# ariasanovsky/azdopt

Measured on AMD Instinct MI355X. Metric: node_expansions_per_s, higher is better.
Workload: dtype f32

## Files before the change

### azdopt_amd/_lib.py

```python
import ctypes as C
import os
import subprocess

_HERE = os.path.dirname(os.path.abspath(__file__))
LIB_PATH = os.environ.get("AZD_LIB", os.path.join(_HERE, "libazdopt_amd.so"))
_LIB = None

CTR = dict(EXPANSIONS=0, TERMINALS=1, TRANSPOSITIONS=2, VISITED_STEPS=3, SELECT_CALLS=4, SUM_DEG=5,
           SUM_ACTIONS=6, CASCADE_NODES=7, NEW_PREDS=8, ROOT_EXHAUSTED=9, MAX_FRONTIER=10, MAX_DEPTH=11,
           CURIOSITY_PAIRS=12, EVAL_LAYER_CLOCKS=13, TICKS_ADD_ACTIONS=14, FAILED=15, TICKS_TOTAL=16, TICKS_SELECT=17, TICKS_LOOKUP=18, TICKS_NEWNODE=19,
           TICKS_CASCADE=20, TICKS_MAX_CALL=21, TICKS_LAMBDA=22, TICKS_MATCHING=23, TICKS_WAIT=24, EVAL_BATCHES=25, EVAL_ROWS=26, EVAL_TILES=27, TICKS_TILES=28, TICKS_BATCH=29, TICKS_TILE_SETUP=30, TICKS_TILE_KLOOP=31)
CTR_COUNT = 32

ACT_NONE, ACT_RELU, ACT_SIGMOID = 0, 1, 2
ENGINE_NO_PERSISTENT_STEP = 1
ENGINE_ASYNC_STEP = 2
ENGINE_BARRIER_STEP = 4
ENGINE_POOL_STEP = 8
ENGINE_DENSE_AH = 32
ENGINE_RAMSEY_U64 = 16
ENGINE_EXT_POOL_STEP = 64
ENGINE_EXT_POOL_F32 = 128
SPACE_C21 = 1
SPACE_RAMSEY = 2
# ... 98 lines not shown
    sig("azd_version", C.c_int)
    sig("azd_device_count", C.c_int)
    sig("azd_c21_state_dim", C.c_int, C.c_int)
    sig("azd_c21_action_dim", C.c_int, C.c_int)
    sig("azd_c21_key_words", C.c_int, C.c_int)
    sig("azd_c21_generate_roots", C.c_int, C.c_uint64, C.c_uint64, C.c_uint64, C.c_int, C.c_int, C.c_int, C.c_int, vp, vp)
    sig("azd_evaluator_create_mlp", C.c_int, C.POINTER(vp), C.c_int, C.c_int, C.c_int, C.c_int, vp, C.c_int, C.c_int,
        C.POINTER(AdamConfig), C.c_uint64)
    sig("azd_evaluator_create_trivial", C.c_int, C.POINTER(vp), C.c_int, C.c_int, C.c_int)
    sig("azd_evaluator_create_hash_stream", C.c_int, C.POINTER(vp), C.c_int, C.c_int, C.c_int, C.c_uint64, C.c_uint64)
    sig("azd_evaluator_destroy", C.c_int, vp)
    sig("azd_evaluator_write_predictions", C.c_int, vp, C.c_int, vp, vp)
    sig("azd_evaluator_update_model", C.c_int, vp, C.c_int, vp, vp, vp, f32p)
    sig("azd_evaluator_write_predictions_dev", C.c_int, vp, C.c_int, vp, vp, vp)
    sig("azd_evaluator_update_model_dev", C.c_int, vp, C.c_int, vp, vp, vp, f32p, vp)
    sig("azd_evaluator_set_weight_storage", C.c_int, vp, C.c_int)
    sig("azd_evaluator_num_params", C.c_int64, vp)
    sig("azd_evaluator_get_params", C.c_int, vp, vp)
    sig("azd_evaluator_set_params", C.c_int, vp, vp)
    sig("azd_evaluator_calls", C.c_uint64, vp)
    sig("azd_engine_create", C.c_int, C.POINTER(vp), C.POINTER(EngineConfig), vp)
    sig("azd_engine_destroy", C.c_int, vp)
    sig("azd_engine_par_new", C.c_int, vp, vp, vp)
    sig("azd_engine_par_roll_out_episodes", C.c_int, vp, vp, C.c_int, C.c_uint32, C.c_int, i32p)
    sig("azd_engine_run_ahead", C.c_int, vp, vp, C.c_int, C.c_uint32, C.c_int, i32p)
    sig("azd_engine_par_update_model", C.c_int, vp, C.c_uint32, f32p)
    sig("azd_engine_par_update_model_sharded", C.c_int, vp, C.c_uint32, vp, f32p)
    sig("azd_engine_par_reset_trees", C.c_int, vp, vp, vp)
    sig("azd_engine_argmin_data", C.c_int, vp, C.POINTER(Argmin))
    sig("azd_engine_agent_counters", C.c_int, vp, vp)
    sig("azd_engine_agent_counters_per_agent", C.c_int, vp)
    sig("azd_engine_pool_agent_finish", C.c_int, vp, vp)
    sig("azd_engine_pool_groups", C.c_int, vp, vp, vp, vp)
    sig("azd_engine_ramsey_argmin_data", C.c_int, vp, C.POINTER(RamseyArgmin))
    sig("azd_engine_ramsey_wide_argmin_data", C.c_int, vp, C.POINTER(RamseyWideArgmin))
    sig("azd_engine_ramsey_argmin_any", C.c_int, vp, vp, C.c_int, vp, C.c_int, vp, f32p, i32p, C.POINTER(C.c_uint32))
    sig("azd_engine_ramsey_agent_counts", C.c_int, vp, C.c_int, vp, vp)
    sig("azd_ramsey_state_dim", C.c_int, C.c_int, C.c_int)
    sig("azd_ramsey_action_dim", C.c_int, C.c_int, C.c_int)
    sig("azd_ramsey_key_words", C.c_int, C.c_int, C.c_int)
    sig("azd_ramsey_generate_roots", C.c_int, C.c_uint64, C.c_uint64, C.c_uint64, C.c_int, C.c_int, C.c_int, C.c_int,
        C.c_int, vp, vp)
    sig("azd_ramsey_generate_roots_weighted", C.c_int, C.c_uint64, C.c_uint64, C.c_uint64, C.c_int, C.c_int, C.c_int, C.c_int,
        C.c_int, vp, vp, vp)
    sig("azd_engine_set_root_policy", C.c_int, vp, C.POINTER(RootPolicy))
    sig("azd_engine_get_root_policy", C.c_int, vp, C.POINTER(RootPolicy))
    sig("azd_root_policy_check", C.c_int, C.c_int, C.c_int, C.POINTER(RootPolicy))
    sig("azd_engine_root_policy_report", C.c_int, vp, vp, vp, vp)
    sig("azd_dense_state_dim", C.c_int, C.c_int)
    sig("azd_dense_action_dim", C.c_int, C.c_int)
    sig("azd_dense_key_words", C.c_int, C.c_int)
    sig("azd_dense_generate_roots", C.c_int, C.c_uint64, C.c_uint64, C.c_uint64, C.c_int, C.c_int, C.c_int, C.c_int, C.c_double, vp, vp)
    sig("azd_engine_dense_argmin_data", C.c_int, vp, C.POINTER(DenseArgmin))
    sig("azd_c21_modify_roots", C.c_int, vp, C.c_uint64, C.c_uint64, C.c_int, C.c_int, vp, vp)
    sig("azd_c21_modify_roots_dev", C.c_int, vp, C.c_uint64, C.c_uint64, C.c_int, C.c_int, vp, vp)
    sig("azd_engine_par_reset_trees_c21", C.c_int, vp, C.c_uint64, C.c_uint64, C.c_int, C.c_int)
    sig("azd_engine_modify_roots_dev", C.c_int, vp, C.c_uint64, C.c_uint64, C.c_int, C.c_int, vp, vp)
    sig("azd_engine_par_reset_trees_policy", C.c_int, vp, C.c_uint64, C.c_uint64, C.c_int, C.c_int)
    sig("azd_engine_par_new_begin", C.c_int, vp, vp, vp)
    sig("azd_engine_par_new_end", C.c_int, vp, vp)
    sig("azd_engine_roll_out_begin", C.c_int, vp, vp, C.c_int, C.c_uint32)
    sig("azd_engine_roll_out_end", C.c_int, vp, vp, i32p)
    sig("azd_engine_reset_begin", C.c_int, vp, vp, vp)
    sig("azd_engine_reset_end", C.c_int, vp, vp)
    sig("azd_engine_observe", C.c_int, vp, C.c_uint32, vp, vp, vp)
    sig("azd_engine_observe_dev", C.c_int, vp, C.c_uint32, C.POINTER(vp), C.POINTER(vp), C.POINTER(vp))
# ... 38 lines not shown
```

### azdopt_amd/csrc/engine.hip

```cpp
#include <hip/hip_runtime.h>

#include <dlfcn.h>

#include <algorithm>
#include <climits>
#include <cstdio>
#include <cstring>
#include <functional>
#include <new>
#include <string>
#include <vector>

#include "../../include/azdopt_amd.h"
#include "c21_host.h"
#include "engine_types.h"
#include "evaluator.h"
#include "space_ops.h"

namespace azd {

thread_local std::string g_last_error;

int hip_fail(hipError_t e, const char *what) {
    g_last_error = std::string(what) + ": " + hipGetErrorString(e);
// ... 200 lines not shown
    static constexpr int EXT_STREAMS = 2;
    static constexpr int EXT_IN_FLIGHT = 4;
    hipStream_t ext_stream[EXT_STREAMS] = {};
    hipGraphExec_t ext_graph[EXT_STREAMS] = {};
    uint64_t ext_graph_layout = 0;
    int ext_graph_n = 0;
    bool ext_unsupported = false;
    bool ext_f32 = false;
    uint64_t ext_unsupported_layout = 0;
    uint32_t *d_ext_rows = nullptr, *d_ext_home = nullptr, *d_ext_n = nullptr;
    unsigned long long *d_ext_t0 = nullptr;
    int ext_depth = 2;
    hipEvent_t ext_done = nullptr, ext_fork = nullptr, ext_ring[EXT_STREAMS][EXT_IN_FLIGHT] = {};
    unsigned long long ext_iterations = 0;
    const struct ExtPoolForm *ext = nullptr;
    uint16_t *ext_s16 = nullptr;
    int ext_s16_pitch = 0;
    int kw_host = 0;
    int ramsey_slots = 0;
    int dense_slots = 0;
    uint64_t *d_stage_slots = nullptr;
    azd_root_policy root_policy{AZD_ROOT_RULE_THRESHOLD, 0, {0.0, 0.0, 0.0, 0.0}};
    azd::RootPolicyArgs root_args{};
    uint32_t *d_root_report = nullptr;
    uint32_t *root_report = nullptr;
    bool root_report_valid = false;
    std::vector<uint64_t> dense_packed;
    std::vector<uint64_t> ramsey_perm_pad;
    bool pool_step = false;
    azd::PoolArgs pool{};
    size_t pool_slot_words = 0;
    int n_cus = 0;
    int pool_eval_wgs = 0, pool_search_wgs = 0;
    int pool_grp_g = 0, pool_grp_groups = 0, pool_grp_w = 0;
    int pool_search_waves = 0;
    double pool_util_eval = 0, pool_util_search = 0;
    struct {
        int n_eval = 0;
        int updates = 0;
    } pool_fb;
    struct Window {
        bool open = false;
        bool drained = false;
        bool lumped = false;
        int n = 0, consumed = 0;
        azd::TolTable tol{};
        uint32_t best_ord = 0;
        unsigned long long best_key = ~0ull;
        unsigned long long side_key = ~0ull;
        unsigned long long base_improved = 0;
        unsigned long long reported = 0;
        azd::FusedEval fe{};
        azd::PoolArgs pool{};
    } win;
    unsigned long long *h_win_log = nullptr;
    uint32_t *h_win_flag = nullptr;
    azd::ArgminRec *d_argmin_side = nullptr;
    azd::RamseyArgminRec *d_argmin_r_side = nullptr;
    bool ramsey_wide() const { return a.space == azd::SPACE_RAMSEY && a.KW > azd::MAX_KW; }
    bool dense_ah() const { return a.space == azd::SPACE_DENSE && a.lam_lo != 0.0; }
    bool ramsey_u64() const { return a.space == azd::SPACE_RAMSEY && a.KW == azd::RAMSEY_U64_KW; }
    size_t ramsey_nbr_words() const { return ramsey_u64() ? 512 : 128; }
    size_t argmin_r_bytes() const {
        return ramsey_u64() ? sizeof(azd::RamseyU64ArgminRec) : ramsey_wide() ? sizeof(azd::RamseyWideArgminRec) : sizeof(azd::RamseyArgminRec);
    }
    size_t argmin_r_recs() const { return (argmin_r_bytes() + sizeof(azd::RamseyArgminRec) - 1) / sizeof(azd::RamseyArgminRec); }
// ... 1412 lines not shown
            e->d_grp_desc = e->d_grp_cnt = nullptr;
            e->d_grp_x = nullptr;
            AZD_HIP(hipMalloc(&e->d_grp_desc, slots * 64 * 4));
            AZD_HIP(hipMalloc(&e->d_grp_cnt, slots * 8 * 32 * 4));
            AZD_HIP(hipMalloc(&e->d_grp_x, slots * 2 * gpl.xstride * 4));
            AZD_HIP(hipMalloc(&e->d_grp_flag, slots * gpl.g * 16 * 4));
            e->grp_flag_words = slots * gpl.g * 16;
            e->grp_slots_alloc = slots;
            e->grp_x_floats = slots * 2 * gpl.xstride;
        }
        if (gpl.tile != e->grp_tile_host || gpl.lds != e->grp_lds_host) {
            AZD_HIP(hipStreamSynchronize(e->stream));
            AZD_HIP(hipMemcpy(e->d_grp_tile, gpl.tile.data(), gpl.tile.size() * sizeof(int16_t), hipMemcpyHostToDevice));
            AZD_HIP(hipMemcpy(e->d_grp_lds, gpl.lds.data(), gpl.lds.size() * sizeof(uint32_t), hipMemcpyHostToDevice));
            e->grp_tile_host = gpl.tile;
            e->grp_lds_host = gpl.lds;
        }
    }
    pool->grp_g = gpl.g;
    pool->grp_w = gpl.W;
    pool->grp_groups = n_groups;
    pool->grp_tile = e->d_grp_tile;
    pool->grp_lds = e->d_grp_lds;
    pool->grp_desc = e->d_grp_desc;
    pool->grp_cnt = e->d_grp_cnt;
    pool->grp_x = e->d_grp_x;
    pool->grp_flag = e->d_grp_flag;
    pool->grp_xstride = gpl.xstride;
    pool->n_eval = n_groups * gpl.g;
    if (gpl.lds_bytes > *dyn_bytes) *dyn_bytes = gpl.lds_bytes;
    return AZD_OK;
}

struct StepPlan {
    azd::FusedEval fe;
    uint32_t dyn_stride;
    size_t dyn_bytes;
    azd::PoolArgs pool;
    int pool_blocks;
    bool feedback;
};

static int plan_step(azd_engine *e, int n_calls, StepPlan *out) {
    StepPlan &p = *out;
    const std::string dense_reason = e->a.space == azd::SPACE_DENSE ? e->step_reason : std::string();
    const bool ext_ramsey = e->ext && e->a.space == azd::SPACE_RAMSEY;
    const std::string ext_reason = ext_ramsey ? e->step_reason : std::string();
    const bool ext_demoted = ext_ramsey && e->pool_failed;
    p.pool = e->pool;
    const bool fusable = e->persist_enabled && !ext_demoted && e->ev->fused_desc(&p.fe);
    const bool pool_wanted = fusable && e->pool_step;
    const char *why_a = "", *why_b = "", *why_p = "";
    const bool pool_planned = pool_wanted && e->ops->pool_plan(e->a, p.fe, &p.pool, &p.dyn_stride, &p.dyn_bytes, &why_p);
    bool use_pool = pool_planned, use_async = false, use_barrier = false;
    e->step_reason.clear();
    if (pool_planned) {
        const int capacity = knob_int("AZD_POOL_MAX_RESIDENT", e->ops->pool_max_resident(e->a, p.dyn_bytes, e->n_cus));
        PoolKnobs k;
        k.eval_wgs = knob_pos("AZD_POOL_EVAL_WGS", 0);
        k.search_wgs = knob_pos("AZD_POOL_SEARCH_WGS", 0);
        k.ready_lanes = knob_int("AZD_POOL_READY_LANES", 0);
        k.express_wgs = knob_int("AZD_POOL_EXPRESS_WGS", KNOB_UNSET);
        k.express_waves = knob_int("AZD_POOL_EXPRESS_WAVES", 8);
        k.express_shift = knob_int("AZD_POOL_EXPRESS_SHIFT", 4);
        k.early_post = knob_int("AZD_POOL_EARLY_POST", KNOB_UNSET);
        const int n_search = pool_split(e->n_cus, e->a, p.fe, n_calls, capacity, pool_feedback_on() ? e->pool_fb.n_eval : 0, k, &p.pool);
        if (n_search < 1 || capacity < 1) {
            use_pool = false;
            char buf[160];
            snprintf(buf, sizeof(buf), "pool step: the device holds %d of its workgroups at once; it needs an evaluator and a searcher resident together; ", capacity);
            e->step_reason = buf;
        }
        p.pool.debug_abort_call = (uint32_t)knob_int("AZD_POOL_DEBUG_ABORT_CALL", 0);
        AZD_ST(ensure_eval_groups(e, p.fe, use_pool, capacity - n_search, knob_int("AZD_POOL_EVAL_GROUP", KNOB_UNSET), &p.pool, &p.dyn_bytes));
        p.pool_blocks = p.pool.n_eval + n_search;
        e->pool_grp_g = p.pool.grp_g;
        e->pool_grp_groups = p.pool.grp_groups;
        e->pool_grp_w = p.pool.grp_w;
        e->pool_eval_wgs = p.pool.n_eval;
        e->pool_search_wgs = n_search;
        e->pool_search_waves = (n_search - p.pool.n_express) * 16 + p.pool.n_express * (int)p.pool.express_waves;
    }
    auto step_down = [&]() {
        use_async = !e->barrier_step && e->ops->async_plan(e->a, p.fe, &p.dyn_stride, &p.dyn_bytes, &why_a);
        use_barrier = !use_async && e->ops->persist_plan(e->a, p.fe, &p.dyn_stride, &p.dyn_bytes, &why_b);
        if (!use_async) e->step_reason += why_a;
        if (!use_async && !use_barrier && *why_b) e->step_reason += std::string("; ") + why_b;
    };
    if (!e->persist_enabled) e->step_reason = "AZD_ENGINE_NO_PERSISTENT_STEP";
    else if (!fusable) e->step_reason = "the evaluator cannot run inside the kernel (external model, more than 7 layers, or a layer width that is not a multiple of 4)";
    else if (pool_planned && !use_pool) step_down();
    else if (!use_pool) {
        if (pool_wanted) e->step_reason = std::string(why_p) + "; ";
        if (e->barrier_step) e->step_reason = "AZD_ENGINE_BARRIER_STEP";
        step_down();
        if (e->pool_failed && use_async)
            e->step_reason = "an earlier pool launch of this engine aborted (a queue wait ran into its bound): asynchronous step";
        if (pool_wanted) step_down();
    }
    e->step_form = use_pool ? AZD_STEP_POOL : use_async ? AZD_STEP_ASYNC : use_barrier ? AZD_STEP_BARRIER : AZD_STEP_PER_CALL;
    p.feedback = use_pool && p.fe.kind == 3 && pool_feedback_on() && !getenv("AZD_POOL_EVAL_WGS");
    if (e->a.space == azd::SPACE_DENSE)
        e->step_reason = dense_reason.empty() ? "AZD_DENSE_NO_POOL: the dense-graph space's pool step was switched off" : dense_reason;
    if (ext_ramsey) e->step_reason = ext_demoted || e->step_reason.empty() ? ext_reason : ext_reason + "; " + e->step_reason;
    return AZD_OK;
}
static void pool_feedback_update(azd_engine *e) {
// ... 978 lines not shown
    AZD_HIP(hipMemcpy(out, e->a.counters, (size_t)e->a.B * azd::NUM_COUNTERS * 8, hipMemcpyDeviceToHost));
    return AZD_OK;
}
int azd_engine_agent_counters_per_agent(azd_engine *e) { return e ? (e->counters_by_wave ? 0 : 1) : AZD_ERR_INVALID_ARGUMENT; }

int azd_engine_set_timing(azd_engine *e, int enabled) {
    if (!e) return AZD_ERR_INVALID_ARGUMENT;
    e->timing = enabled != 0;
    e->rollout_ms = e->evaluator_ms = 0;
    e->rollout_launches = 0;
    return AZD_OK;
}
int azd_engine_timing(azd_engine *e, double *tree_ms, double *evaluator_ms, uint64_t *tree_launches) {
    if (!e) return AZD_ERR_INVALID_ARGUMENT;
    if (tree_ms) *tree_ms = e->rollout_ms;
    if (evaluator_ms) *evaluator_ms = e->evaluator_ms;
    if (tree_launches) *tree_launches = e->rollout_launches;
    return AZD_OK;
}
void *azd_engine_stream(azd_engine *e) { return e ? (void *)e->stream : nullptr; }
int azd_engine_pool_utilisation(azd_engine *e, double *eval_busy, double *search_busy) {
    if (!e) return AZD_ERR_INVALID_ARGUMENT;
    if (eval_busy) *eval_busy = e->pool_util_eval;
    if (search_busy) *search_busy = e->pool_util_search;
    return AZD_OK;
}
int azd_engine_pool_groups(azd_engine *e, int *members, int *groups, int *waves_per_slot) {
    if (!e) return AZD_ERR_INVALID_ARGUMENT;
    if (members) *members = e->pool_grp_g;
    if (groups) *groups = e->pool_grp_groups;
    if (waves_per_slot) *waves_per_slot = e->pool_grp_w;
    return AZD_OK;
}
int azd_engine_pool_agent_finish(azd_engine *e, uint64_t *ticks_out) {
    if (!e || !ticks_out) return AZD_ERR_INVALID_ARGUMENT;
    AZD_ENTER(e);
    if (!e->pool.stamp) {
        azd::g_last_error = "pool_agent_finish: this engine has run no pool step";
        return AZD_ERR_INVALID_ARGUMENT;
    }
    AZD_HIP(hipStreamSynchronize(e->stream));
    AZD_HIP(hipMemcpy(ticks_out, e->pool.stamp, (size_t)e->a.B * 8, hipMemcpyDeviceToHost));
    return AZD_OK;
}
int azd_engine_pool_split(azd_engine *e, int *eval_wgs, int *search_wgs) {
    if (!e) return AZD_ERR_INVALID_ARGUMENT;
    if (eval_wgs) *eval_wgs = e->pool_eval_wgs;
    if (search_wgs) *search_wgs = e->pool_search_wgs;
    return AZD_OK;
}
int azd_debug_probe_xcc(int device, uint32_t *out, int n_blocks) {
    if (!out || n_blocks <= 0) return AZD_ERR_INVALID_ARGUMENT;
    AZD_ST(azd::device_ok(device));
    AZD_HIP(hipSetDevice(device));
    uint32_t *d = nullptr;
    AZD_HIP(hipMalloc(&d, (size_t)n_blocks * 4));
    azd::launch_probe_xcc(d, n_blocks, nullptr);
    hipError_t he = hipDeviceSynchronize();
    if (he == hipSuccess) he = hipMemcpy(out, d, (size_t)n_blocks * 4, hipMemcpyDeviceToHost);
    (void)hipFree(d);
    if (he != hipSuccess) return azd::hip_fail(he, "probe_xcc");
    return AZD_OK;
}
int azd_debug_ext_pool_plan(const azd_engine_config *cfg, int *waves, size_t *lds_bytes) {
    if (!cfg || !waves || !lds_bytes) return AZD_ERR_INVALID_ARGUMENT;
    AZD_ST(check_engine_config(cfg));
// ... 255 lines not shown
```

### azdopt_amd/csrc/engine_types.h

```cpp
#pragma once
#include <stddef.h>
#include <stdint.h>

namespace azd {

constexpr uint32_t NONE = 0xFFFFFFFFu;
constexpr int PARENTS_STRIDE = 32;
constexpr int MAX_N = 24;
constexpr int MAX_KW = 6;
constexpr int PATH_SET = 0, PATH_SEQUENCE = 1;
constexpr int SPACE_C21 = 1, SPACE_RAMSEY = 2, SPACE_DENSE = 3;
constexpr int PRED_CHUNKS = 2;
constexpr int MAX_NODE_ACTIONS = 64 * PRED_CHUNKS;
constexpr int RAMSEY_U64_KW = 36;
constexpr int RAMSEY_U64_CH = 8;
constexpr int FRONTIER_CAP = 256;
constexpr int PATH_STACK = 32;
constexpr int MAX_TOL = 32;
constexpr int NUM_COUNTERS = 32;

struct __attribute__((aligned(16))) NodeRec {
    float c_star;
    uint32_t nt_ex;
    float c;
// ... 227 lines not shown
    uint32_t n_preds;
    uint32_t call;
};
struct PoolArgs {
    PoolCtl *ctl;
    uint32_t *ready_slots;
    uint32_t *eval_slots;
    int ready_lanes;
    int n_express;
    uint32_t express_waves;
    uint32_t express_shift;
    int early_post;
    uint32_t qcap;
    uint32_t *join;
    PendRec *pend;
    unsigned long long *stamp;
    int n_eval;
    uint32_t eval_stride;
    uint32_t eval_out_off;
    uint32_t eval_rows;
    uint32_t *post_call;
    int grp_g, grp_w, grp_groups;
    const int16_t *grp_tile;
    const uint32_t *grp_lds;
    uint32_t *grp_desc;
    uint32_t *grp_cnt;
    uint32_t *grp_flag;
    float *grp_x;
    uint32_t grp_xstride;
    uint32_t debug_abort_call;
    uint32_t *win_count;
    unsigned long long *win_log;
    uint32_t *win_flag;
};

struct StepLaunch {
    int n_calls;
    unsigned long long *log_key;
    const uint32_t *resume;
    PoolCtl *ctl;
    int hashed;
    int groups = 0;
    int window;
};

struct PersistArgs {
    Arenas a;
    TolTable tol;
    FusedEval ev;
    PoolArgs pool;
};

}
```

### azdopt_amd/csrc/pool_step.inc

```

constexpr unsigned long long POOL_WAIT_TICKS = 400000000ull;
struct PoolWait {
    unsigned long long t0;
    uint32_t polls;
    __device__ __forceinline__ PoolWait() : t0(0), polls(0) {}
    __device__ __forceinline__ bool expired() {
        if ((++polls & 255u) != 0u) return false;
        const unsigned long long now = (unsigned long long)wall_clock64();
        if (t0 == 0) t0 = now;
        return now - t0 > POOL_WAIT_TICKS;
    }
};

__device__ __forceinline__ uint32_t pool_xcc_id() {
    uint32_t v;
    asm volatile("s_getreg_b32 %0, hwreg(HW_REG_XCC_ID)" : "=s"(v));
    return v & 7u;
}

#ifndef AZD_POOL_FILL_WAIT
#define AZD_POOL_FILL_WAIT 2
#endif
#ifndef AZD_POOL_FILL_SLEEP
#define AZD_POOL_FILL_SLEEP 32
// ... 155 lines not shown
            tile_k_loop_bf16(acc, reinterpret_cast<const uint16_t *>(gp.wpk) + tile0, (uint32_t)lane * 8u,
                             (uint32_t)(uintptr_t)(reinterpret_cast<const uint16_t *>(rbase) + in_off), steps);
        else
            tile_k_loop_f32(acc, reinterpret_cast<const float *>(gp.wpk) + tile0, (uint32_t)lane * 16u, (uint32_t)(uintptr_t)(rbase + in_off), steps);
    }
    const int lane = opaque_lane();
    const int col = n0 + (lane & 15);
    if (col < N) {
        const float bj = gp.params[ev.b_off[l] + col];
        const int act = (l == L - 1) ? ev.final_act : 1;
#pragma unroll
        for (int i = 0; i < 4; ++i) {
            const int row = 4 * (lane >> 4) + i;
            if (row < nrows) {
                const float v = act_apply(acc[i] + bj, act);
                if (l == L - 1) rows.out(row)[col] = v;
                else if (ev.bf16) reinterpret_cast<uint16_t *>(rows.row(row))[S4 + (l & 1) * H + col] = (uint16_t)bf16_bits(v);
                else rows.row(row)[S4 + (l & 1) * H + col] = v;
            }
        }
    }
}

__device__ __forceinline__ void pool_hash_rows(const FusedEval &ev, const PoolArgs &pl, const PoolBatch &bt, const PoolRows &rows, const int n,
                                            const int A) {
    for (int idx = threadIdx.x; idx < n * A; idx += PERSIST_WAVES * 64) {
        const int r = idx / A, i = idx - r * A;
        const uint64_t agent = ev.first_agent + (uint64_t)bt.agent[r], cidx = ev.call_base + (uint64_t)ld_sc1(pl.post_call + bt.agent[r]);
        const uint64_t h = splitmix(splitmix(splitmix(splitmix(ev.seed ^ 0x70726564ull) ^ agent) ^ cidx) ^ (uint64_t)i);
        rows.out(r)[i] = (float)(h >> 40) * (1.0f / 16777216.0f);
    }
}

template <bool HASHED>
__device__ __forceinline__ void pool_eval(const PersistArgs *pa, const EvalPtrs &gp, PoolBatch &bt, const uint32_t xcc) {
    const Arenas &a = pa->a;
    const FusedEval &ev = pa->ev;
    const PoolArgs &pl = pa->pool;
    PoolCtl *ctl = pl.ctl;
    const int tid = threadIdx.x, wave = tid >> 6;
    const uint32_t B = (uint32_t)a.B, qmask = pl.qcap - 1u;
    constexpr bool hashed = HASHED;
    const int S = ev.dims[0], S16 = (S + 15) & ~15, L = hashed ? 0 : ev.n_layers, A = hashed ? a.A : ev.dims[L];
    PoolRows rows;
    rows.stride = pl.eval_stride;
    rows.out_off = pl.eval_out_off;
    rows.agents = bt.agent;
    unsigned long long n_batches = 0, n_rows = 0, n_tiles = 0, busy = 0, t_stage = 0, t_layers = 0, c_layers = 0;
    for (;;) {
        if (tid == 0) {
            uint32_t n = 0, first0 = 0, first1 = 0, cnt0 = 0, cnt1 = 0, q = 0, leave = 0;
            PoolWait wt;
            int fill_waits = AZD_POOL_FILL_WAIT;
            for (;;) {
                for (uint32_t k = 0; k < (uint32_t)POOL_XCDS && n == 0u; ++k) {
                    const uint32_t x = (xcc + k) & (uint32_t)(POOL_XCDS - 1);
                    const uint32_t h0 = AZD_POOL_PRIORITY ? ld_sc1(&ctl->evalq[0][x].head) : 0u, t0 = AZD_POOL_PRIORITY ? ld_sc1(&ctl->evalq[0][x].tail) : 0u;
                    const uint32_t h1 = ld_sc1(&ctl->evalq[1][x].head), t1 = ld_sc1(&ctl->evalq[1][x].tail);
                    const int a0 = (int)(t0 - h0) > 0 ? (int)(t0 - h0) : 0, a1 = (int)(t1 - h1) > 0 ? (int)(t1 - h1) : 0;
                    if (a0 + a1 == 0) continue;
                    const int cap = ((int)pl.eval_rows > PERSIST_WAVES && a0 + a1 >= (int)pl.eval_rows) ? (int)pl.eval_rows : PERSIST_WAVES;
                    if (a0 == 0 && a1 < PERSIST_WAVES && fill_waits > 0) {
                        --fill_waits;
                        __builtin_amdgcn_s_sleep(AZD_POOL_FILL_SLEEP);
                        k = (uint32_t)POOL_XCDS;
                        continue;
                    }
                    uint32_t c0 = 0, c1 = 0;
                    if (a0 > 0) {
                        const uint32_t take = a0 < cap ? (uint32_t)a0 : (uint32_t)cap;
                        if (atomicCAS(&ctl->evalq[0][x].head, h0, h0 + take) == h0) c0 = take;
                    }
                    if (a1 > 0 && c0 < (uint32_t)cap) {
                        const uint32_t room = (uint32_t)cap - c0;
                        const uint32_t take = (uint32_t)a1 < room ? (uint32_t)a1 : room;
                        if (atomicCAS(&ctl->evalq[1][x].head, h1, h1 + take) == h1) c1 = take;
                    }
                    if (c0 + c1) {
                        n = c0 + c1;
                        first0 = h0;
                        first1 = h1;
                        cnt0 = c0;
// ... 43 lines not shown
            bt.agent[tid] = v ? (v & 0xFFFFFFu) - 1u : 0u;
            bt.home[tid] = v >> 24;
#ifdef AZD_PHASE_PROFILE
            if (v) {
                unsigned long long *st = pl.stamp + bt.agent[tid];
                atomicAdd(&a.counters[(size_t)bt.agent[tid] * NUM_COUNTERS + 24], (unsigned long long)wall_clock64() - __hip_atomic_load(st, __ATOMIC_RELAXED, __HIP_MEMORY_SCOPE_AGENT));
            }
#endif
        }
        __syncthreads();
        if (bt.leave) break;
        rows.n = n;
        if (hashed) pool_hash_rows(ev, pl, bt, rows, n, A);
        else {
            const int q4 = S16 >> 2;
            for (int idx = tid; idx < n * q4; idx += PERSIST_WAVES * 64) {
                const int r = idx / q4, c4 = idx - r * q4;
                azd_f32x4 v = {0.f, 0.f, 0.f, 0.f};
                if (4 * c4 < S) v = ld_sc1_x4(gp.state_vecs + (size_t)bt.agent[r] * S + 4 * c4);
                if (ev.bf16) {
                    uint16_t *d = reinterpret_cast<uint16_t *>(rows.row(r)) + 4 * c4;
                    d[0] = (uint16_t)bf16_bits(v[0]);
                    d[1] = (uint16_t)bf16_bits(v[1]);
                    d[2] = (uint16_t)bf16_bits(v[2]);
                    d[3] = (uint16_t)bf16_bits(v[3]);
                } else *reinterpret_cast<azd_f32x4 *>(rows.row(r) + 4 * c4) = v;
            }
        }
        __syncthreads();
        const unsigned long long tb1 = (unsigned long long)wall_clock64();
        const unsigned long long cb1 = (unsigned long long)__builtin_amdgcn_s_memtime();
        for (int l = 0; l < L; ++l) {
            const int nt = (ev.dims[l + 1] + 15) >> 4;
            for (int tile = wave; tile < nt; tile += PERSIST_WAVES) {
                if (n > PERSIST_WAVES) {
                    if (ev.bf16) pool_tile2<true>(ev, rows, gp, l, tile);
                    else pool_tile2<false>(ev, rows, gp, l, tile);
                } else {
#if AZD_POOL_ASM_TILE
                    pool_tile1(ev, rows, gp, l, tile);
#else
                    unsigned long long ph[3];
                    mlp_tile_task<PoolRows, true>(ev, rows, gp, l, tile, ph);
#endif
                }
            }
            __syncthreads();
        }
        for (int l = 0; l < L; ++l) n_tiles += (unsigned long long)((ev.dims[l + 1] + 15) >> 4);
        const unsigned long long tb2 = (unsigned long long)wall_clock64();
        t_stage += tb1 - tb0;
        t_layers += tb2 - tb1;
        c_layers += (unsigned long long)__builtin_amdgcn_s_memtime() - cb1;
        {
            const int a4 = A >> 2;
            for (int idx = tid; idx < n * a4; idx += PERSIST_WAVES * 64) {
                const int r = idx / a4, c4 = idx - r * a4;
                st_sc1_x4(gp.h_theta + (size_t)bt.agent[r] * A + 4 * c4, *reinterpret_cast<const azd_f32x4 *>(rows.out(r) + 4 * c4));
            }
        }
        VM_DRAIN();
        __syncthreads();
        if (tid < n && ((bt.home[tid] & 0x40u) == 0u || (atomicAdd(&pl.join[bt.agent[tid]], 1u) & 1u))) {
#ifdef AZD_PHASE_PROFILE
            __hip_atomic_store(pl.stamp + bt.agent[tid], (unsigned long long)wall_clock64(), __ATOMIC_RELAXED, __HIP_MEMORY_SCOPE_AGENT);
#endif
            const uint32_t x = bt.home[tid] & (uint32_t)(POOL_XCDS - 1);
            const uint32_t rl = (pl.ready_lanes && (bt.home[tid] & 0x80u)) ? 0u : 1u;
            const uint32_t i = atomicAdd(&ctl->ready[rl][x].tail, 1u);
            st_sc1(pl.ready_slots + ((size_t)rl * POOL_XCDS + x) * pl.qcap + (i & qmask), bt.agent[tid] + 1u);
        }
        n_batches += 1;
        n_rows += (unsigned long long)n;
        if (tid == 0 && blockIdx.x == 0 && pl.debug_abort_call != 0u && n_batches == (unsigned long long)pl.debug_abort_call) atomicExch(&ctl->abort, 1u);
        busy += (unsigned long long)wall_clock64() - tb0;
    }
    if (tid == 0) {
        atomicAdd(&ctl->eval_busy, busy);
        atomicMax(&ctl->t_last, (unsigned long long)wall_clock64());
        unsigned long long *ctr = a.counters + (size_t)(blockIdx.x % (uint32_t)a.B) * NUM_COUNTERS;
        atomicAdd(&ctr[25], n_batches);
        atomicAdd(&ctr[26], n_rows);
        atomicAdd(&ctr[27], n_tiles);
        atomicAdd(&ctr[29], busy);
#ifndef AZD_PHASE_PROFILE
        atomicAdd(&ctr[30], t_stage);
        atomicAdd(&ctr[31], t_layers);
#endif
        atomicAdd(&ctr[13], c_layers);
    }
}

struct GroupTile {
    int tile;
    uint32_t lds;
};
__device__ __forceinline__ azd_f32x4 grp_buf_ld(__amdgpu_buffer_rsrc_t r, uint32_t byte_off) {
    typedef unsigned int u32x4 __attribute__((ext_vector_type(4)));
    const u32x4 v = __builtin_amdgcn_raw_buffer_load_b128(r, byte_off, 0, 16);
    azd_f32x4 f;
    __builtin_memcpy(&f, &v, 16);
    return f;
}
__device__ __forceinline__ void pool_eval_group(const PersistArgs *pa, const EvalPtrs &gp, const uint32_t xcc) {
    const Arenas &a = pa->a;
    const FusedEval &ev = pa->ev;
    const PoolArgs &pl = pa->pool;
    PoolCtl *ctl = pl.ctl;
    const int lane = LANE, wave = threadIdx.x >> 6;
    const int g = pl.grp_g, W = pl.grp_w, NS = PERSIST_WAVES / W;
// ... 770 lines not shown
```

### azdopt_amd/optimizer.py

```python
import ctypes as C

import numpy as np

from . import _lib
from .space import ActionSet


class ArgminData:

    def __init__(self, rec, n, kw):
        self.state = dict(parents=np.array(rec.parents[:n], np.uint8), permitted=np.array(rec.permitted[:kw], np.uint64))
        m = rec.matching_size
        self.cost = dict(lambda_1=rec.lambda_1, matching=[(rec.matching[2 * i], rec.matching[2 * i + 1]) for i in range(m)])
        self.eval = np.float32(rec.eval)
        self.agent, self.node = rec.agent, rec.node


class RamseyArgminData:

    def __init__(self, rec, space):
        self.state = dict(colors=np.array(rec.colors[:space.E], np.uint8), permitted=np.array(rec.permitted[:], np.uint64))
        self.cost = dict(clique_counts=[int(x) for x in rec.totals[:space.C]])
        self.eval = np.float32(rec.eval)
        self.agent, self.node = rec.agent, rec.node
# ... 295 lines not shown
    def ramsey_argmin_any(self):
        import types
        E = self.space.E
        colors, permitted, totals = np.zeros(E, np.uint8), np.zeros((E + 63) // 64, np.uint64), np.zeros(4, np.int32)
        ev, agent, node = C.c_float(), C.c_int32(), C.c_uint32()
        _lib.check(self._L.azd_engine_ramsey_argmin_any(self._h, _lib.ptr(colors), E, _lib.ptr(permitted), len(permitted), _lib.ptr(totals),
                                                         C.byref(ev), C.byref(agent), C.byref(node)), "ramsey_argmin_any")
        return types.SimpleNamespace(colors=colors, permitted=permitted, totals=totals, eval=ev.value, agent=agent.value, node=node.value)

    def ramsey_agent_counts(self, agent):
        counts = np.zeros((self.space.C, self.space.E), np.int32)
        totals = np.zeros(4, np.int32)
        _lib.check(self._L.azd_engine_ramsey_agent_counts(self._h, agent, _lib.ptr(counts), _lib.ptr(totals)), "ramsey_agent_counts")
        return counts, totals[:self.space.C]

    def counters(self):
        out = np.zeros(_lib.CTR_COUNT, np.uint64)
        _lib.check(self._L.azd_engine_counters(self._h, _lib.ptr(out)), "counters")
        return {k: int(out[v]) for k, v in _lib.CTR.items()}

    def agent_counters(self, allow_wave_blocks=False):
        if not allow_wave_blocks and self._L.azd_engine_agent_counters_per_agent(self._h) == 0:
            raise RuntimeError("agent_counters: the pool step of the product build attributes counters to searcher waves, not agents "
                               "(use counters() for the sums, the PROFILE build or pool_step=False for per-agent values)")
        out = np.zeros((self.batch, _lib.CTR_COUNT), np.uint64)
        _lib.check(self._L.azd_engine_agent_counters(self._h, _lib.ptr(out)), "agent_counters")
        return {k: out[:, v].copy() for k, v in _lib.CTR.items()}

    def pool_groups(self):
        g, n, w = C.c_int(), C.c_int(), C.c_int()
        _lib.check(self._L.azd_engine_pool_groups(self._h, C.byref(g), C.byref(n), C.byref(w)), "pool_groups")
        return g.value, n.value, w.value

    def pool_agent_finish_ms(self):
        out = np.zeros(self.batch, np.uint64)
        _lib.check(self._L.azd_engine_pool_agent_finish(self._h, _lib.ptr(out)), "pool_agent_finish")
        return out.astype(np.float64) * 1e-5

    def set_timing(self, enabled=True):
        _lib.check(self._L.azd_engine_set_timing(self._h, int(enabled)), "set_timing")

    def timing(self):
        a, b, n = C.c_double(), C.c_double(), C.c_uint64()
        _lib.check(self._L.azd_engine_timing(self._h, C.byref(a), C.byref(b), C.byref(n)), "timing")
        return dict(rollout_ms=a.value, evaluator_ms=b.value, rollout_launches=n.value)

    def stream(self):
        return self._L.azd_engine_stream(self._h)

    STEP_FORMS = {0: "none", 1: "async", 2: "barrier", 3: "per_call", 4: "pool", 5: "per_call_graph"}

    def pool_split(self):
        a, b = C.c_int32(), C.c_int32()
        _lib.check(self._L.azd_engine_pool_split(self._h, C.byref(a), C.byref(b)), "pool_split")
        return a.value, b.value

    def pool_utilisation(self):
        a, b = C.c_double(), C.c_double()
        _lib.check(self._L.azd_engine_pool_utilisation(self._h, C.byref(a), C.byref(b)), "pool_utilisation")
        return a.value, b.value

    def step_form(self):
        form, why = C.c_int32(), C.c_char_p()
        _lib.check(self._L.azd_engine_step_form(self._h, C.byref(form), C.byref(why)), "step_form")
        return self.STEP_FORMS.get(form.value, "?"), (why.value or b"").decode()
```

### include/azdopt_amd.h

```cpp
#ifndef AZDOPT_AMD_H
#define AZDOPT_AMD_H
#include <stdint.h>
#ifdef __cplusplus
extern "C" {
#endif

typedef enum azd_status {
    AZD_OK = 0,
    AZD_ERR_INVALID_ARGUMENT = 1,
    AZD_ERR_NO_DEVICE = 2,
    AZD_ERR_HIP = 3,
    AZD_ERR_CAPACITY = 4,
    AZD_ERR_UNREACHABLE = 5,
    AZD_ERR_NO_EVALUATOR = 6,
    AZD_ERR_OUT_OF_MEMORY = 7,
    AZD_ERR_UNSUPPORTED = 8
} azd_status;

const char *azd_status_string(int status);
const char *azd_last_error(void);
int azd_version(void);
int azd_device_count(void);

#define AZD_SPACE_C21 1
// ... 224 lines not shown
int azd_engine_roll_out_end(azd_engine *e, const float *h_theta, int *improved);
int azd_engine_reset_begin(azd_engine *e, const uint8_t *parents, const uint64_t *permitted);
int azd_engine_reset_end(azd_engine *e, const float *h_theta);
int azd_engine_observe(azd_engine *e, uint32_t n_obs_tol, float *state_vecs, float *observations,
                       float *action_weights);
int azd_engine_observe_dev(azd_engine *e, uint32_t n_obs_tol, const float **d_state_vecs,
                           const float **d_observations, const float **d_action_weights);
int azd_engine_read_state_vecs(azd_engine *e, float *state_vecs);
int azd_engine_read_predictions(azd_engine *e, float *h_theta);
int azd_engine_debug_tile_forward(azd_engine *e, const float *states, float *predictions, int rows);

int azd_engine_tree_sizes(azd_engine *e, int agent, int *n_nodes, int *n_arcs, int *n_predictions);
int azd_engine_export_tree(azd_engine *e, int agent, float *c, float *c_star, uint32_t *n_t,
                           uint32_t *exhausted, uint32_t *act_begin, uint32_t *act_end,
                           uint64_t *keys, uint32_t *arc_src, uint32_t *arc_dst, uint32_t *arc_pp,
                           uint32_t *pred_a_id, float *pred_g, int32_t *pred_arc);
int azd_engine_agent_state(azd_engine *e, int agent, uint8_t *parents, uint64_t *permitted,
                           uint64_t *path, uint32_t *state_pos, double *lambda_1,
                           int *matching_size);
int azd_engine_counters(azd_engine *e, uint64_t *out );
int azd_engine_agent_counters(azd_engine *e, uint64_t *out);
int azd_engine_agent_counters_per_agent(azd_engine *e);
int azd_engine_set_timing(azd_engine *e, int enabled);
int azd_engine_timing(azd_engine *e, double *tree_ms, double *evaluator_ms, uint64_t *tree_launches);
void *azd_engine_stream(azd_engine *e);
#define AZD_STEP_NONE 0
#define AZD_STEP_ASYNC 1
#define AZD_STEP_BARRIER 2
#define AZD_STEP_PER_CALL 3
#define AZD_STEP_POOL 4
#define AZD_STEP_PER_CALL_GRAPH 5
int azd_engine_step_form(azd_engine *e, int *form, const char **reason);
int azd_engine_pool_groups(azd_engine *e, int *members, int *groups, int *waves_per_slot);
int azd_engine_pool_agent_finish(azd_engine *e, uint64_t *ticks_out);
int azd_engine_pool_split(azd_engine *e, int *eval_wgs, int *search_wgs);
int azd_engine_pool_utilisation(azd_engine *e, double *eval_busy, double *search_busy);
int azd_debug_probe_xcc(int device, uint32_t *out, int n_blocks);
int azd_debug_hash_stream_via_evaluators(azd_evaluator *ev, int on);
int azd_debug_ext_pool_plan(const azd_engine_config *cfg, int *waves, size_t *lds_bytes);
int azd_debug_write_predictions_gathered(azd_evaluator *ev, int max_rows, const uint32_t *rows, int n_rows, const float *states,
                                         int n_state_rows, float *predictions);
int azd_debug_mlp_gradients(azd_evaluator *ev, int batch, const float *states, const float *observations,
                            const float *action_weights, float *grads_out, float *loss);

int azd_debug_probe_math(int device, const float *in, float *out, int n);
int azd_debug_probe_cost(int device, const uint8_t *parents, int n, int count, int reps, int full,
                         double *lambda_1, int *matching_size, float *ms);

#define AZD_DENSE_AH_MAX_N 32
typedef struct azd_dense_ah_cost_t {
    double proximity;
    double eigenvalue;
    int32_t diameter;
    int32_t k;
    float cost;
    float eval;
} azd_dense_ah_cost_t;
int azd_dense_ah_cost(const uint64_t *adj, int n, azd_dense_ah_cost_t *out);
int azd_debug_probe_ah_cost(int device, const uint64_t *adj, int n, int count, int reps, azd_dense_ah_cost_t *out, float *ms);
typedef struct azd_dense_ah_argmin {
    uint64_t adj[32];
    uint64_t permitted[8];
    double proximity, eigenvalue;
    int32_t diameter, k;
    float cost, eval;
    int32_t agent;
// ... 14 lines not shown
```

Baseline: 39.04 million.

## Keep largest MLP layer weights register-resident in pool evaluator waves

Each pool evaluator wave now loads the weight fragments of its tile for the largest one or two MLP layers into VGPRs once, at kernel start, and reuses them for every batch. The weights are no longer re-streamed from global memory on each layer pass. A planner picks the layers and can be switched off through the AZD_POOL_EVAL_RESIDENT knob. The register array raises VGPR pressure and can lower occupancy, and the resident path covers only one tile per wave instead of striding over tiles.

Result: slower. 38.54 million (-1.3%).

```diff
diff --git a/azdopt_amd/_lib.py b/azdopt_amd/_lib.py
--- a/azdopt_amd/_lib.py
+++ b/azdopt_amd/_lib.py
@@ -154,6 +154,8 @@
     sig("azd_engine_agent_counters_per_agent", C.c_int, vp)
     sig("azd_engine_pool_agent_finish", C.c_int, vp, vp)
     sig("azd_engine_pool_groups", C.c_int, vp, vp, vp, vp)
+    sig("azd_engine_pool_resident", C.c_int, vp, vp, vp, vp)
+    sig("azd_pool_resident_plan", C.c_int, i32p, C.c_int, C.c_int, i32p, i32p, i32p)
     sig("azd_engine_ramsey_argmin_data", C.c_int, vp, C.POINTER(RamseyArgmin))
     sig("azd_engine_ramsey_wide_argmin_data", C.c_int, vp, C.POINTER(RamseyWideArgmin))
     sig("azd_engine_ramsey_argmin_any", C.c_int, vp, vp, C.c_int, vp, C.c_int, vp, f32p, i32p, C.POINTER(C.c_uint32))
diff --git a/azdopt_amd/csrc/engine.hip b/azdopt_amd/csrc/engine.hip
--- a/azdopt_amd/csrc/engine.hip
+++ b/azdopt_amd/csrc/engine.hip
@@ -256,6 +256,7 @@
     size_t pool_slot_words = 0;
     int n_cus = 0;
     int pool_eval_wgs = 0, pool_search_wgs = 0;
+    int pool_res_layer[2] = {-1, -1}, pool_res_ksteps = 0;
     int pool_grp_g = 0, pool_grp_groups = 0, pool_grp_w = 0;
     int pool_search_waves = 0;
     double pool_util_eval = 0, pool_util_search = 0;
@@ -1734,6 +1735,39 @@
     return AZD_OK;
 }
 
+static void pool_resident_layers(const int *dims, int n_layers, bool bf16, int out[2]) {
+    out[0] = out[1] = -1;
+    long long best[2] = {0, 0};
+    for (int l = 0; l < n_layers; ++l) {
+        const int K = dims[l], N = dims[l + 1];
+        if (K < 1 || N < 1 || (K + 15) / 16 > azd::POOL_RES_MAX_KSTEPS || (N + 15) / 16 > 16) continue;
+        const long long bytes = (long long)K * N;
+        if (bytes > best[0]) {
+            best[1] = best[0];
+            out[1] = out[0];
+            best[0] = bytes;
+            out[0] = l;
+        } else if (bytes > best[1]) {
+            best[1] = bytes;
+            out[1] = l;
+        }
+    }
+    if (!bf16) out[1] = -1;
+}
+static int pool_resident_plan(const int *dims, int n_layers, bool bf16, int out[2], int *ksteps) {
+    const int knob = knob_int("AZD_POOL_EVAL_RESIDENT", 1);
+    if (knob != 0 && knob != 1) {
+        azd::g_last_error = "AZD_POOL_EVAL_RESIDENT must be 0 (every layer streamed) or 1 (resident layer: the default)";
+        return AZD_ERR_INVALID_ARGUMENT;
+    }
+    out[0] = out[1] = -1;
+    if (knob) pool_resident_layers(dims, n_layers, bf16, out);
+    *ksteps = 0;
+    for (int i = 0; i < 2; ++i)
+        if (out[i] >= 0) *ksteps = std::max(*ksteps, std::min((dims[out[i]] + 15) / 16, azd::POOL_RES_KSTEPS));
+    return AZD_OK;
+}
+
 struct StepPlan {
     azd::FusedEval fe;
     uint32_t dyn_stride;
@@ -1775,6 +1809,13 @@
         }
         p.pool.debug_abort_call = (uint32_t)knob_int("AZD_POOL_DEBUG_ABORT_CALL", 0);
         AZD_ST(ensure_eval_groups(e, p.fe, use_pool, capacity - n_search, knob_int("AZD_POOL_EVAL_GROUP", KNOB_UNSET), &p.pool, &p.dyn_bytes));
+        p.pool.res_layer[0] = p.pool.res_layer[1] = -1;
+        p.pool.res_ksteps = 0;
+        if (use_pool && p.fe.kind == 3 && p.pool.grp_g == 0)
+            AZD_ST(pool_resident_plan(p.fe.dims, p.fe.n_layers, p.fe.bf16 != 0, p.pool.res_layer, &p.pool.res_ksteps));
+        e->pool_res_layer[0] = p.pool.res_layer[0];
+        e->pool_res_layer[1] = p.pool.res_layer[1];
+        e->pool_res_ksteps = p.pool.res_ksteps;
         p.pool_blocks = p.pool.n_eval + n_search;
         e->pool_grp_g = p.pool.grp_g;
         e->pool_grp_groups = p.pool.grp_groups;
@@ -2819,6 +2860,21 @@
     if (waves_per_slot) *waves_per_slot = e->pool_grp_w;
     return AZD_OK;
 }
+int azd_engine_pool_resident(azd_engine *e, int *layer0, int *layer1, int *ksteps) {
+    if (!e) return AZD_ERR_INVALID_ARGUMENT;
+    if (layer0) *layer0 = e->pool_res_layer[0];
+    if (layer1) *layer1 = e->pool_res_layer[1];
+    if (ksteps) *ksteps = e->pool_res_ksteps;
+    return AZD_OK;
+}
+int azd_pool_resident_plan(const int *dims, int n_layers, int bf16, int *layer0, int *layer1, int *ksteps) {
+    if (!dims || n_layers < 1 || n_layers > 7 || !layer0 || !layer1 || !ksteps) return AZD_ERR_INVALID_ARGUMENT;
+    int out[2];
+    AZD_ST(pool_resident_plan(dims, n_layers, bf16 != 0, out, ksteps));
+    *layer0 = out[0];
+    *layer1 = out[1];
+    return AZD_OK;
+}
 int azd_engine_pool_agent_finish(azd_engine *e, uint64_t *ticks_out) {
     if (!e || !ticks_out) return AZD_ERR_INVALID_ARGUMENT;
     AZD_ENTER(e);
diff --git a/azdopt_amd/csrc/engine_types.h b/azdopt_amd/csrc/engine_types.h
--- a/azdopt_amd/csrc/engine_types.h
+++ b/azdopt_amd/csrc/engine_types.h
@@ -283,7 +283,14 @@
     uint32_t *win_count;
     unsigned long long *win_log;
     uint32_t *win_flag;
-};
+    int res_layer[2];
+    int res_ksteps;
+};
+#ifndef AZD_POOL_RES_KSTEPS
+#define AZD_POOL_RES_KSTEPS 8
+#endif
+constexpr int POOL_RES_KSTEPS = AZD_POOL_RES_KSTEPS;
+constexpr int POOL_RES_MAX_KSTEPS = 16;
 
 struct StepLaunch {
     int n_calls;
diff --git a/azdopt_amd/csrc/pool_step.inc b/azdopt_amd/csrc/pool_step.inc
--- a/azdopt_amd/csrc/pool_step.inc
+++ b/azdopt_amd/csrc/pool_step.inc
@@ -211,13 +211,185 @@
     }
 }
 
+constexpr int POOL_RES_WORDS = 4 * POOL_RES_KSTEPS;
+constexpr int POOL_RES_TAIL = POOL_RES_MAX_KSTEPS - POOL_RES_KSTEPS;
+static_assert(POOL_RES_KSTEPS % 4 == 0 && POOL_RES_KSTEPS >= 4 && POOL_RES_TAIL >= 0 && POOL_RES_TAIL <= 8, "the tail is one group of requests");
+template <bool BF16, int SLOT>
+__device__ __forceinline__ void pool_res_load(const FusedEval &ev, const EvalPtrs &gp, const int l, const int tile, uint32_t (&w)[POOL_RES_WORDS]) {
+    const int steps = (ev.dims[l] + 15) >> 4;
+    const size_t frag = (size_t)ev.p_off[l] + ((size_t)tile * steps * 64 + LANE) * 4;
+    if constexpr (BF16) {
+        const uint16_t *wq = reinterpret_cast<const uint16_t *>(gp.wpk) + frag;
+#pragma unroll
+        for (int s = 0; s < POOL_RES_KSTEPS; ++s)
+            if (s < steps) {
+                const uint2 v = *reinterpret_cast<const uint2 *>(wq + 256 * s);
+                w[2 * (SLOT * POOL_RES_KSTEPS + s)] = v.x;
+                w[2 * (SLOT * POOL_RES_KSTEPS + s) + 1] = v.y;
+            }
+    } else {
+        const float *wp = reinterpret_cast<const float *>(gp.wpk) + frag;
+#pragma unroll
+        for (int s = 0; s < POOL_RES_KSTEPS; ++s)
+            if (s < steps) {
+                const uint4 v = *reinterpret_cast<const uint4 *>(wp + 256 * s);
+                w[4 * s] = v.x;
+                w[4 * s + 1] = v.y;
+                w[4 * s + 2] = v.z;
+                w[4 * s + 3] = v.w;
+            }
+    }
+}
+template <bool TWO>
+__device__ __forceinline__ void pool_res_step_f32(f32x4 &acc0, f32x4 &acc1, const float4 a0, const float4 a1, const float bx, const float by,
+                                                  const float bz, const float bw) {
+    acc0 = __builtin_amdgcn_mfma_f32_16x16x4f32(a0.x, bx, acc0, 0, 0, 0);
+    if constexpr (TWO) acc1 = __builtin_amdgcn_mfma_f32_16x16x4f32(a1.x, bx, acc1, 0, 0, 0);
+    acc0 = __builtin_amdgcn_mfma_f32_16x16x4f32(a0.y, by, acc0, 0, 0, 0);
+    if constexpr (TWO) acc1 = __builtin_amdgcn_mfma_f32_16x16x4f32(a1.y, by, acc1, 0, 0, 0);
+    acc0 = __builtin_amdgcn_mfma_f32_16x16x4f32(a0.z, bz, acc0, 0, 0, 0);
+    if constexpr (TWO) acc1 = __builtin_amdgcn_mfma_f32_16x16x4f32(a1.z, bz, acc1, 0, 0, 0);
+    acc0 = __builtin_amdgcn_mfma_f32_16x16x4f32(a0.w, bw, acc0, 0, 0, 0);
+    if constexpr (TWO) acc1 = __builtin_amdgcn_mfma_f32_16x16x4f32(a1.w, bw, acc1, 0, 0, 0);
+}
+template <bool TWO>
+__device__ __forceinline__ void pool_res_step_bf16(f32x4 &acc0, f32x4 &acc1, const uint2 a0, const uint2 a1, const uint2 bv) {
+    bf16x4 x0, x1, b4;
+    __builtin_memcpy(&x0, &a0, 8);
+    __builtin_memcpy(&x1, &a1, 8);
+    __builtin_memcpy(&b4, &bv, 8);
+    acc0 = __builtin_amdgcn_mfma_f32_16x16x16bf16_1k(x0, b4, acc0, 0, 0, 0);
+    if constexpr (TWO) acc1 = __builtin_amdgcn_mfma_f32_16x16x16bf16_1k(x1, b4, acc1, 0, 0, 0);
+}
+template <bool BF16, int SLOT, bool TWO>
+__device__ __forceinline__ void pool_tile_res(const FusedEval &ev, const PoolRows &rows, const EvalPtrs &gp, const int l, const int tile,
+                                              const uint32_t (&w)[POOL_RES_WORDS]) {
+    constexpr int G = TWO ? 2 : 4;
+    const int lane = opaque_lane();
+    const int L = ev.n_layers;
+    const int K = ev.dims[l], N = ev.dims[l + 1];
+    const int S4 = (ev.dims[0] + 15) & ~15, H = ev.hid[0];
+    const int nrows = rows.count();
+    const int r = lane & 15;
+    float *const base0 = rows.row(r < nrows ? r : 0);
+    float *const base1 = rows.row(TWO && 16 + r < nrows ? 16 + r : 0);
+    const int in_off = (l == 0 ? 0 : S4 + ((l - 1) & 1) * H) + 4 * (lane >> 4);
+    const int steps = (K + 15) >> 4;
+    [[maybe_unused]] const size_t frag = (size_t)ev.p_off[l] + ((size_t)tile * steps * 64 + lane) * 4;
+    f32x4 acc0 = {0.f, 0.f, 0.f, 0.f}, acc1 = {0.f, 0.f, 0.f, 0.f};
+    if constexpr (BF16) {
+        const uint16_t *p0 = reinterpret_cast<const uint16_t *>(base0) + in_off, *p1 = reinterpret_cast<const uint16_t *>(base1) + in_off;
+        [[maybe_unused]] uint2 bq[POOL_RES_TAIL > 0 ? POOL_RES_TAIL : 1];
+        if constexpr (POOL_RES_TAIL > 0) {
+            const uint16_t *wq = reinterpret_cast<const uint16_t *>(gp.wpk) + frag;
+#pragma unroll
+            for (int j = 0; j < POOL_RES_TAIL; ++j)
+                bq[j] = *reinterpret_cast<const uint2 *>(wq + 256 * (POOL_RES_KSTEPS + j < steps ? POOL_RES_KSTEPS + j : steps - 1));
+            __builtin_amdgcn_sched_barrier(0);
+        }
+#pragma unroll
+        for (int g = 0; g < POOL_RES_MAX_KSTEPS; g += G) {
+            if (g >= steps) break;
+            const bool full = g + G <= steps;
+            uint2 a0[G], a1[G];
+#pragma unroll
+            for (int j = 0; j < G; ++j)
+                if (full || g + j < steps) {
+                    a0[j] = *reinterpret_cast<const uint2 *>(p0 + 16 * (g + j));
+                    if constexpr (TWO) a1[j] = *reinterpret_cast<const uint2 *>(p1 + 16 * (g + j));
+                }
+#pragma unroll
+            for (int j = 0; j < G; ++j)
+                if (full || g + j < steps) {
+                    uint2 bv;
+                    if constexpr (POOL_RES_TAIL > 0) {
+                        if (g + j >= POOL_RES_KSTEPS) bv = bq[g + j >= POOL_RES_KSTEPS ? g + j - POOL_RES_KSTEPS : 0];
+                    }
+                    if (g + j < POOL_RES_KSTEPS) {
+                        const int i = 2 * (SLOT * POOL_RES_KSTEPS + (g + j < POOL_RES_KSTEPS ? g + j : 0));
+                        bv = uint2{w[i], w[i + 1]};
+                    }
+                    pool_res_step_bf16<TWO>(acc0, acc1, a0[j], TWO ? a1[j] : a0[j], bv);
+                }
+        }
+    } else {
+        const float *p0 = base0 + in_off, *p1 = base1 + in_off;
+        [[maybe_unused]] float4 bq[POOL_RES_TAIL > 0 ? POOL_RES_TAIL : 1];
+        if constexpr (POOL_RES_TAIL > 0) {
+            const float *wp = reinterpret_cast<const float *>(gp.wpk) + frag;
+#pragma unroll
+            for (int j = 0; j < POOL_RES_TAIL; ++j)
+                bq[j] = *reinterpret_cast<const float4 *>(wp + 256 * (POOL_RES_KSTEPS + j < steps ? POOL_RES_KSTEPS + j : steps - 1));
+            __builtin_amdgcn_sched_barrier(0);
+        }
+#pragma unroll
+        for (int g = 0; g < POOL_RES_MAX_KSTEPS; g += G) {
+            if (g >= steps) break;
+            const bool full = g + G <= steps;
+            float4 a0[G], a1[G];
+#pragma unroll
+            for (int j = 0; j < G; ++j)
+                if (full || g + j < steps) {
+                    a0[j] = *reinterpret_cast<const float4 *>(p0 + 16 * (g + j));
+                    if constexpr (TWO) a1[j] = *reinterpret_cast<const float4 *>(p1 + 16 * (g + j));
+                }
+#pragma unroll
+            for (int j = 0; j < G; ++j)
+                if (full || g + j < steps) {
+                    float bx, by, bz, bw;
+                    if constexpr (POOL_RES_TAIL > 0) {
+                        if (g + j >= POOL_RES_KSTEPS) {
+                            const float4 t = bq[g + j >= POOL_RES_KSTEPS ? g + j - POOL_RES_KSTEPS : 0];
+                            bx = t.x, by = t.y, bz = t.z, bw = t.w;
+                        }
+                    }
+                    if (g + j < POOL_RES_KSTEPS) {
+                        const int i = 4 * (g + j < POOL_RES_KSTEPS ? g + j : 0);
+                        bx = __builtin_bit_cast(float, w[i]), by = __builtin_bit_cast(float, w[i + 1]);
+                        bz = __builtin_bit_cast(float, w[i + 2]), bw = __builtin_bit_cast(float, w[i + 3]);
+                    }
+                    pool_res_step_f32<TWO>(acc0, acc1, a0[j], TWO ? a1[j] : a0[j], bx, by, bz, bw);
+                }
+        }
+    }
+    const int lane2 = opaque_lane();
+    const int col = tile * 16 + (lane2 & 15);
+    if (col < N) {
+        const float bj = gp.params[ev.b_off[l] + col];
+        const int act = (l == L - 1) ? ev.final_act : 1;
+#pragma unroll
+        for (int h = 0; h < (TWO ? 2 : 1); ++h)
+#pragma unroll
+            for (int i = 0; i < 4; ++i) {
+                const int row = 16 * h + 4 * (lane2 >> 4) + i;
+                if (row < nrows) {
+                    const float v = act_apply((h ? acc1[i] : acc0[i]) + bj, act);
+                    if (l == L - 1) rows.out(row)[col] = v;
+                    else if (BF16) reinterpret_cast<uint16_t *>(rows.row(row))[S4 + (l & 1) * H + col] = (uint16_t)bf16_bits(v);
+                    else rows.row(row)[S4 + (l & 1) * H + col] = v;
+                }
+            }
+    }
+}
+template <int SLOT>
+__device__ __forceinline__ void pool_layer_res(const FusedEval &ev, const PoolRows &rows, const EvalPtrs &gp, const int l, const int tile, const int n,
+                                               const uint32_t (&w)[POOL_RES_WORDS]) {
+    if (ev.bf16) {
+        if (n > PERSIST_WAVES) pool_tile_res<true, SLOT, true>(ev, rows, gp, l, tile, w);
+        else pool_tile_res<true, SLOT, false>(ev, rows, gp, l, tile, w);
+    } else if constexpr (SLOT == 0) {
+        if (n > PERSIST_WAVES) pool_tile_res<false, 0, true>(ev, rows, gp, l, tile, w);
+        else pool_tile_res<false, 0, false>(ev, rows, gp, l, tile, w);
+    }
+}
+
 template <bool HASHED>
 __device__ __forceinline__ void pool_eval(const PersistArgs *pa, const EvalPtrs &gp, PoolBatch &bt, const uint32_t xcc) {
     const Arenas &a = pa->a;
     const FusedEval &ev = pa->ev;
     const PoolArgs &pl = pa->pool;
     PoolCtl *ctl = pl.ctl;
-    const int tid = threadIdx.x, wave = tid >> 6;
+    const int tid0 = threadIdx.x, wave0 = tid0 >> 6;
     const uint32_t B = (uint32_t)a.B, qmask = pl.qcap - 1u;
     constexpr bool hashed = HASHED;
     const int S = ev.dims[0], S16 = (S + 15) & ~15, L = hashed ? 0 : ev.n_layers, A = hashed ? a.A : ev.dims[L];
@@ -226,7 +398,27 @@
     rows.out_off = pl.eval_out_off;
     rows.agents = bt.agent;
     unsigned long long n_batches = 0, n_rows = 0, n_tiles = 0, busy = 0, t_stage = 0, t_layers = 0, c_layers = 0;
+    uint32_t wres[POOL_RES_WORDS];
+    int res0 = -1, res1 = -1;
+    if constexpr (!hashed) {
+        if (pl.res_ksteps > 0) {
+            res0 = pl.res_layer[0];
+            res1 = pl.res_layer[1];
+        }
+#pragma unroll
+        for (int i = 0; i < POOL_RES_WORDS; ++i) wres[i] = 0u;
+        if (res0 >= 0 && wave0 < ((ev.dims[res0 + 1] + 15) >> 4)) {
+            if (ev.bf16) pool_res_load<true, 0>(ev, gp, res0, wave0, wres);
+            else pool_res_load<false, 0>(ev, gp, res0, wave0, wres);
+        }
+        if (res1 >= 0 && wave0 < ((ev.dims[res1 + 1] + 15) >> 4)) pool_res_load<true, 1>(ev, gp, res1, wave0, wres);
+#pragma unroll
+        for (int i = 0; i < POOL_RES_WORDS; ++i) asm volatile("" : "+v"(wres[i]));
+    }
     for (;;) {
+        int tid = tid0;
+        asm volatile("" : "+v"(tid));
+        const int wave = __builtin_amdgcn_readfirstlane(tid >> 6);
         if (tid == 0) {
             uint32_t n = 0, first0 = 0, first1 = 0, cnt0 = 0, cnt1 = 0, q = 0, leave = 0;
             PoolWait wt;
@@ -336,7 +528,19 @@
         const unsigned long long cb1 = (unsigned long long)__builtin_amdgcn_s_memtime();
         for (int l = 0; l < L; ++l) {
             const int nt = (ev.dims[l + 1] + 15) >> 4;
-            for (int tile = wave; tile < nt; tile += PERSIST_WAVES) {
+            int wl = wave;
+            asm volatile("" : "+s"(wl));
+            bool resident = false;
+            if constexpr (!hashed) {
+                if (l == res0) {
+                    resident = true;
+                    if (wl < nt) pool_layer_res<0>(ev, rows, gp, l, wl, n, wres);
+                } else if (l == res1) {
+                    resident = true;
+                    if (wl < nt) pool_layer_res<1>(ev, rows, gp, l, wl, n, wres);
+                }
+            }
+            for (int tile = wl; tile < nt && !resident; tile += PERSIST_WAVES) {
                 if (n > PERSIST_WAVES) {
                     if (ev.bf16) pool_tile2<true>(ev, rows, gp, l, tile);
                     else pool_tile2<false>(ev, rows, gp, l, tile);
@@ -379,7 +583,7 @@
         if (tid == 0 && blockIdx.x == 0 && pl.debug_abort_call != 0u && n_batches == (unsigned long long)pl.debug_abort_call) atomicExch(&ctl->abort, 1u);
         busy += (unsigned long long)wall_clock64() - tb0;
     }
-    if (tid == 0) {
+    if (tid0 == 0) {
         atomicAdd(&ctl->eval_busy, busy);
         atomicMax(&ctl->t_last, (unsigned long long)wall_clock64());
         unsigned long long *ctr = a.counters + (size_t)(blockIdx.x % (uint32_t)a.B) * NUM_COUNTERS;
diff --git a/azdopt_amd/optimizer.py b/azdopt_amd/optimizer.py
--- a/azdopt_amd/optimizer.py
+++ b/azdopt_amd/optimizer.py
@@ -351,6 +351,11 @@
         _lib.check(self._L.azd_engine_pool_groups(self._h, C.byref(g), C.byref(n), C.byref(w)), "pool_groups")
         return g.value, n.value, w.value
 
+    def pool_resident(self):
+        a, b, k = C.c_int(), C.c_int(), C.c_int()
+        _lib.check(self._L.azd_engine_pool_resident(self._h, C.byref(a), C.byref(b), C.byref(k)), "pool_resident")
+        return a.value, b.value, k.value
+
     def pool_agent_finish_ms(self):
         out = np.zeros(self.batch, np.uint64)
         _lib.check(self._L.azd_engine_pool_agent_finish(self._h, _lib.ptr(out)), "pool_agent_finish")
diff --git a/include/azdopt_amd.h b/include/azdopt_amd.h
--- a/include/azdopt_amd.h
+++ b/include/azdopt_amd.h
@@ -280,6 +280,8 @@
 #define AZD_STEP_PER_CALL_GRAPH 5
 int azd_engine_step_form(azd_engine *e, int *form, const char **reason);
 int azd_engine_pool_groups(azd_engine *e, int *members, int *groups, int *waves_per_slot);
+int azd_engine_pool_resident(azd_engine *e, int *layer0, int *layer1, int *ksteps);
+int azd_pool_resident_plan(const int *dims, int n_layers, int bf16, int *layer0, int *layer1, int *ksteps);
 int azd_engine_pool_agent_finish(azd_engine *e, uint64_t *ticks_out);
 int azd_engine_pool_split(azd_engine *e, int *eval_wgs, int *search_wgs);
 int azd_engine_pool_utilisation(azd_engine *e, double *eval_busy, double *search_busy);
```
